# JoshFCooper415/differential_transformer_replication

Measured on AMD Instinct MI355X. Metric: diff-attn fwd+bwd TFLOP/s (% MFMA peak); train tokens/sec at 1/2/4/8 GPUs, higher is better.
Workload: dtype bf16; 1 GPU; cfg2: fused N=2 diff-attention core fwd+bwd (BASELINE configs[1]); batch_per_gpu=8, global_batch=8, heads=16, head_size=64, dv=128, seq_len=4096, n_terms=2, causal=True, parallelism=batch-sharded replicas x1 (no data-path collective)

## Files before the change

### differential_transformer_replication_amd/csrc/attn_kernels.h

```cpp
#pragma once
#include "dta_common.h"
#include "dta_internal.h"
#include "layout_checks.h"

#include <type_traits>
#include <utility>

#ifndef DTA_STAMPS
#define DTA_STAMPS 0
#endif

namespace dta {

template <int NSEG_ = 8>
struct Stamps {
  static constexpr int NSEG = NSEG_;
  unsigned t = 0, s[NSEG] = {};
  __device__ __forceinline__ static unsigned now() {
    unsigned long long v;
    __builtin_amdgcn_sched_barrier(0);
    asm volatile("s_memtime %0\n\ts_waitcnt lgkmcnt(0)" : "=s"(v) : : "memory");
    __builtin_amdgcn_sched_barrier(0);
    return (unsigned)v;
  }
  __device__ __forceinline__ void start() { if constexpr (DTA_STAMPS) t = now(); }
  template <int J>
  __device__ __forceinline__ void lap() {
    if constexpr (DTA_STAMPS) {
      const unsigned n = now();
      s[J] += n - t;
      t = n;
    }
  }
  __device__ __forceinline__ void flush(unsigned long long* out, int wave_id, int lane) {
    if constexpr (DTA_STAMPS) {
      if (out && lane == 0)
#pragma unroll
        for (int j = 0; j < 8; ++j) out[(int64_t)wave_id * 8 + j] = j < NSEG ? s[j] : 0;
    }
  }
};

constexpr int img_cols(int c) {
  int p = 1;
  while (p < c) p <<= 1;
  return p;
}

template <int ROWB>
__device__ __forceinline__ int swz(int r) {
  if constexpr (ROWB >= 256) return ((r & 3) << 2) | ((r >> 2) & 3);
  else if constexpr (ROWB == 128) return (((r >> 1) & 1) << 2) | ((r >> 2) & 3);
  else if constexpr (ROWB == 64) return (r >> 2) & 3;
  else return (r >> 3) & 1;
}

template <class E, int COLS>
struct Img {
  static constexpr int ES = (int)sizeof(E);
  static constexpr int ROWB = COLS * ES;
  static constexpr int CPR = ROWB / 16;
  static_assert(ROWB >= 32 && (ROWB & (ROWB - 1)) == 0, "image rows must be a power of two >= 32 B");
  __device__ static int off(int r, int col) {
    const int byte = col * ES;
    return (r * ROWB + ((((byte >> 4) ^ swz<ROWB>(r)) << 4) | (byte & 15))) / ES;
  }
  using O = Ops<E>;
  using frag = typename O::frag;
  __device__ static frag row(const E* img, int r, int s, int h) {
    if constexpr (ES == 2) return *reinterpret_cast<const frag*>(img + off(r, s * 16 + h * 8));
    else return img[off(r, 2 * s + h)];
  }
  template <class V4>
  __device__ static V4 tr4(const E* img, int r0, int cbase, int lane) {
    const int i = lane & 15;
    const E* p = img + off(r0 + (i >> 2), cbase + ((lane >> 4) & 1) * 16 + (i & 3) * 4);
    s16x4 v = __builtin_amdgcn_ds_read_tr16_b64_v4i16((lds_s16x4*)(p));
    return __builtin_bit_cast(V4, v);
  }
  __device__ static frag tr_perm(const E* img, int rbase, int s, int h, int cbase, int lane) {
    if constexpr (ES == 2) {
      typedef E v4 __attribute__((ext_vector_type(4)));
      v4 lo = tr4<v4>(img, rbase + 16 * s + 4 * h, cbase, lane);
      v4 hi = tr4<v4>(img, rbase + 16 * s + 8 + 4 * h, cbase, lane);
      return __builtin_shufflevector(lo, hi, 0, 1, 2, 3, 4, 5, 6, 7);
    } else {
      return img[off(rbase + (s & 3) + 8 * (s >> 2) + 4 * h, cbase + (lane & 31))];
    }
  }
};

__device__ __forceinline__ void rope_inv4(const float* rope, int64_t row, int hs, int e, float& a0, float& a1,
                                          float& a2, float& a3) {
  const f32x4 t = *reinterpret_cast<const f32x4*>(rope + (row * (hs >> 1) + (e >> 1)) * 2);
  const float b0 = fmaf(a0, t[0], a1 * t[1]), b1 = fmaf(a1, t[0], -a0 * t[1]);
  const float b2 = fmaf(a2, t[2], a3 * t[3]), b3 = fmaf(a3, t[2], -a2 * t[3]);
  a0 = b0; a1 = b1; a2 = b2; a3 = b3;
}

__device__ __forceinline__ uint32_t fmix32(uint32_t x) {
  x ^= x >> 16; x *= 0x85ebca6bu; x ^= x >> 13; x *= 0xc2b2ae35u; x ^= x >> 16;
  return x;
}
__device__ __forceinline__ uint32_t drop_key(uint32_t seed_lo, uint32_t seed_hi, int b, int h, int i, int H, int N) {
  return fmix32(seed_lo ^ fmix32((uint32_t)((b * H + h) * N + i) + seed_hi));
}
__device__ __forceinline__ float drop_mul(uint32_t key, int q, int k, uint32_t thr, float scale) {
  const uint32_t x = fmix32((key + (uint32_t)q * 0x9e3779b1u) ^ ((uint32_t)k * 0x7feb352du));
  return x >= thr ? scale : 0.f;
}

template <class F, int... I>
__device__ __forceinline__ void sfor_impl(F&& f, std::integer_sequence<int, I...>) {
  (f(std::integral_constant<int, I>{}), ...);
}
template <int N, class F>
__device__ __forceinline__ void sfor(F&& f) { sfor_impl(f, std::make_integer_sequence<int, N>{}); }

__device__ __forceinline__ unsigned lds_addr(const void* p) {
  return (unsigned)(uintptr_t)(const __attribute__((address_space(3))) char*)(p);
}

template <int ROWB>
__device__ __forceinline__ int tr_lane(int lane) {
  const int h = (lane >> 5) & 1, i = lane & 15, q = i >> 2;
  const int y = ((lane >> 4) & 1) * 2 + ((i & 3) >> 1);
  int L = (4 * h + q) * ROWB + 16 * (y ^ h) + 8 * (i & 1);
  if constexpr (ROWB >= 256) L += 64 * q;
  else if constexpr (ROWB == 128) L += 64 * (q >> 1);
  return L;
}
template <int ROWB>
__device__ __forceinline__ int row_lane(int lane) {
  const int c = lane & 31, h = (lane >> 5) & 1;
  return c * ROWB + 16 * (h ^ swz<ROWB>(c));
}

typedef long long lds64;
template <int ROWB, int RB, int OFF = 0>
__device__ __forceinline__ void tr_issue(lds64 (&r)[4], unsigned a0, unsigned a1) {
  static_assert(OFF + ROWB * (RB + 24) < 65536, "DS immediate offset");
  asm volatile(
      "ds_read_b64_tr_b16 %0, %4 offset:%6\n\t"
      "ds_read_b64_tr_b16 %1, %5 offset:%7\n\t"
      "ds_read_b64_tr_b16 %2, %4 offset:%8\n\t"
      "ds_read_b64_tr_b16 %3, %5 offset:%9"
      : "=&v"(r[0]), "=&v"(r[1]), "=&v"(r[2]), "=&v"(r[3])
      : "v"(a0), "v"(a1), "i"(OFF + ROWB * RB), "i"(OFF + ROWB * (RB + 8)), "i"(OFF + ROWB * (RB + 16)),
        "i"(OFF + ROWB * (RB + 24)));
}
__device__ __forceinline__ const __attribute__((address_space(3))) char* lds_ptr(unsigned a) {
  return reinterpret_cast<const __attribute__((address_space(3))) char*>((size_t)a);
}
template <class T>
__device__ __forceinline__ T lds_at(unsigned a, int off) {
  return *reinterpret_cast<const __attribute__((address_space(3))) T*>(lds_ptr(a) + off);
}
template <int M>
__device__ __forceinline__ void lgkm_pin(lds64 (&r)[M][4]) {
  asm volatile("s_waitcnt lgkmcnt(0)" ::: "memory");
#pragma unroll
  for (int m = 0; m < M; ++m)
#pragma unroll
    for (int j = 0; j < 4; ++j) asm volatile("" : "+v"(r[m][j]));
}
typedef int i32x4 __attribute__((ext_vector_type(4)));
template <int OFF>
__device__ __forceinline__ void ds128(i32x4& r, unsigned a) {
  static_assert(OFF >= 0 && OFF < 65536, "DS immediate offset");
  asm volatile("ds_read_b128 %0, %1 offset:%2" : "=v"(r) : "v"(a), "i"(OFF));
}
template <int N>
__device__ __forceinline__ void lgkm_wait() {
  asm volatile("s_waitcnt lgkmcnt(%0)" ::"i"(N) : "memory");
}

#ifndef DTA_FWD_PIPE
#define DTA_FWD_PIPE 3
#endif
#ifndef DTA_DQ_PIPE
#define DTA_DQ_PIPE 3
#endif
static_assert(DTA_FWD_PIPE >= 1 && DTA_FWD_PIPE <= 15, "DTA_FWD_PIPE: 1 .. 15 reads ahead");
static_assert(DTA_DQ_PIPE >= 1 && DTA_DQ_PIPE <= 15, "DTA_DQ_PIPE: 1 .. 15 reads ahead");

template <class E, int NSQ, int NKB, int QL, int D, int KOFF, int QOFF, int KROWB>
__device__ __forceinline__ void s_chain_pipe(f32x16 (&sa)[NKB], unsigned bK, unsigned bQ,
                                             const typename Ops<E>::frag* qreg) {
  using frag = typename Ops<E>::frag;
  constexpr int PER = NKB + QL, NR = NSQ * PER;
  constexpr bool KBIG = KOFF + NKB * 32 * KROWB >= 65536, QBIG = QOFF + 1024 >= 65536;
  bK += KBIG ? KOFF : 0;
  bQ += QBIG ? QOFF : 0;
  i32x4 kr[D + 1], qv[QL ? NSQ : 1];
  auto issue = [&](auto J) {
    constexpr int j = decltype(J)::value, st = j / PER, w = j % PER;
    if constexpr (QL && w == 0) ds128<(QBIG ? 0 : QOFF)>(qv[QL ? st : 0], bQ ^ (32 * st));
    else ds128<(KBIG ? 0 : KOFF) + (w - QL) * 32 * KROWB>(kr[(st * NKB + w - QL) % (D + 1)], bK ^ (32 * st));
  };
  sfor<(D < NR ? D : NR)>([&](auto J) { issue(J); });
  sfor<NSQ * NKB>([&](auto C) {
    constexpr int c = decltype(C)::value, st = c / NKB, kb = c % NKB;
    constexpr int j = st * PER + QL + kb;
    constexpr int from = c == 0 ? D : ((c - 1) / NKB) * PER + QL + (c - 1) % NKB + D + 1;
    sfor<NR>([&](auto J2) {
      constexpr int j2 = decltype(J2)::value;
      if constexpr (j2 >= from && j2 <= j + D) issue(std::integral_constant<int, j2>{});
    });
    constexpr int issued = (j + D + 1 < NR ? j + D + 1 : NR);
    lgkm_wait<issued - 1 - j>();
    asm volatile("" : "+v"(kr[c % (D + 1)]));
    frag qb;
    if constexpr (QL) {
      asm volatile("" : "+v"(qv[QL ? st : 0]));
      qb = __builtin_bit_cast(frag, qv[QL ? st : 0]);
    } else {
      qb = qreg[st];
    }
    sa[kb] = Ops<E>::mma(__builtin_bit_cast(frag, kr[c % (D + 1)]), qb, sa[kb]);
  });
}

template <int CNT, int M>
__device__ __forceinline__ void lgkm_pin_n(lds64 (&r)[M][4]) {
  asm volatile("s_waitcnt lgkmcnt(%0)" ::"i"(CNT) : "memory");
#pragma unroll
  for (int m = 0; m < M; ++m)
#pragma unroll
    for (int j = 0; j < 4; ++j) asm volatile("" : "+v"(r[m][j]));
}

template <int ROWB, int RB, int OFF = 0>
__device__ __forceinline__ void tr_load(lds64 (&r)[4], unsigned a0, unsigned a1) {
  typedef short v4s __attribute__((ext_vector_type(4)));
  auto rd = [](unsigned a) {
    return __builtin_bit_cast(lds64, __builtin_amdgcn_ds_read_tr16_b64_v4i16(
        reinterpret_cast<__attribute__((address_space(3))) v4s*>((size_t)a)));
  };
  r[0] = rd(a0 + OFF + ROWB * RB);
  r[1] = rd(a1 + OFF + ROWB * (RB + 8));
  r[2] = rd(a0 + OFF + ROWB * (RB + 16));
  r[3] = rd(a1 + OFF + ROWB * (RB + 24));
}

template <class E>
__device__ __forceinline__ typename Ops<E>::frag tr_frag(const lds64 (&r)[4], int s) {
  typedef short v4s __attribute__((ext_vector_type(4)));
  const v4s lo = __builtin_bit_cast(v4s, r[2 * s]), hi = __builtin_bit_cast(v4s, r[2 * s + 1]);
  return __builtin_bit_cast(typename Ops<E>::frag, __builtin_shufflevector(lo, hi, 0, 1, 2, 3, 4, 5, 6, 7));
}

template <class E, int COLS, int ROWS, int VALID, int NTHR>
__device__ __forceinline__ void stage(E* img, const E* g, int64_t rs, int row0, int rowmax, int tid) {
  using I = Img<E, COLS>;
  constexpr int BYTES = ROWS * I::ROWB;
  if constexpr (VALID == COLS && BYTES % 1024 == 0) {
    constexpr int NI = BYTES / 1024;
    const int wave = tid >> 6, lane = tid & 63;
#pragma unroll
    for (int j0 = 0; j0 < NI; j0 += NTHR / 64) {
      const int j = j0 + wave;
      if (NI % (NTHR / 64) == 0 || j < NI) {
        const int pb = j * 1024 + lane * 16;
        const int r = pb / I::ROWB;
        const int c = ((pb % I::ROWB) >> 4) ^ swz<I::ROWB>(r);
        const int row = min(row0 + r, rowmax);
        const char* src = reinterpret_cast<const char*>(g + (int64_t)row * rs) + c * 16;
        __builtin_amdgcn_global_load_lds(src, (__attribute__((address_space(3))) void*)(reinterpret_cast<char*>(img) + j * 1024),
                                         16, 0, 0);
      }
    }
  } else {
    constexpr int CH = ROWS * I::CPR;
    for (int c = tid; c < CH; c += NTHR) {
      const int r = c / I::CPR, ch = c % I::CPR;
      const int row = row0 + r;
      const bool ok = row <= rowmax && ch * 16 < VALID * I::ES;
      s16x8 v = ok ? *reinterpret_cast<const s16x8*>(reinterpret_cast<const char*>(g + (int64_t)row * rs) + ch * 16)
                   : s16x8{};
      *reinterpret_cast<s16x8*>(reinterpret_cast<char*>(img) + r * I::ROWB + ((ch ^ swz<I::ROWB>(r)) << 4)) = v;
    }
  }
}

template <class E>
__device__ __forceinline__ void rope_frag(typename Ops<E>::frag& f, const float* fr, int t, int col, int HS, int hf) {
  if constexpr (sizeof(E) == 2) {
    const float* q = fr + ((int64_t)t * (HS / 2) + col / 2) * 2;
    const f32x4 a = *reinterpret_cast<const f32x4*>(q), b = *reinterpret_cast<const f32x4*>(q + 4);
    const float cs[4] = {a[0], a[2], b[0], b[2]}, sn[4] = {a[1], a[3], b[1], b[3]};
#pragma unroll
    for (int j = 0; j < 4; ++j) {
      const float x = (float)f[2 * j], y = (float)f[2 * j + 1];
      f[2 * j] = (E)(x * cs[j] - y * sn[j]);
      f[2 * j + 1] = (E)(x * sn[j] + y * cs[j]);
    }
  } else {
    const float* q = fr + ((int64_t)t * (HS / 2) + col / 2) * 2;
    const float c = q[0], sn = q[1];
    const float other = __shfl_xor(f, 32, 64);
    f = hf == 0 ? f * c - other * sn : other * sn + f * c;
  }
}
template <class E, int COLS, int ROWS, int VALID, int NTHR>
__device__ __forceinline__ void rope_lds(E* img, const float* fr, int row0, int T, E* gout, int64_t ors, bool write,
                                         int tid) {
  using I = Img<E, COLS>;
  constexpr int V = 16 / (int)sizeof(E);
  typedef E vec __attribute__((ext_vector_type(V)));
  for (int x = tid; x < ROWS * I::CPR; x += NTHR) {
    const int r = x / I::CPR, ch = x % I::CPR;
    if (ch * V >= VALID) continue;
    const int t = min(row0 + r, T - 1);
    vec* a = reinterpret_cast<vec*>(reinterpret_cast<char*>(img) + r * I::ROWB + ((ch ^ swz<I::ROWB>(r)) << 4));
    vec v = *a;
    const float* q = fr + ((int64_t)t * (VALID / 2) + ch * V / 2) * 2;
#pragma unroll
    for (int j = 0; j < V / 2; ++j) {
      const float c = q[2 * j], sn = q[2 * j + 1];
      const float xx = (float)v[2 * j], yy = (float)v[2 * j + 1];
      v[2 * j] = (E)(xx * c - yy * sn);
      v[2 * j + 1] = (E)(xx * sn + yy * c);
    }
    *a = v;
    if (write && row0 + r < T) *reinterpret_cast<vec*>(gout + (int64_t)(row0 + r) * ors + ch * V) = v;
  }
}

template <class E, int NTHR>
__device__ __forceinline__ void scale_lds(E* a, int n, float s, int tid) {
  constexpr int V = 16 / (int)sizeof(E);
  typedef E vec __attribute__((ext_vector_type(V)));
  for (int e = tid * V; e < n; e += NTHR * V) {
    vec x = *reinterpret_cast<vec*>(a + e);
#pragma unroll
    for (int j = 0; j < V; ++j) x[j] = (E)((float)x[j] * s);
    *reinterpret_cast<vec*>(a + e) = x;
  }
}

template <int N, int NR, int NTHR>
__device__ __forceinline__ void stage_rows(float* dst, const float* src, int64_t bs, int row0, int rowmax, int tid) {
  constexpr int TOT = N * NR;
  constexpr int NI = (TOT + 63) / 64;
  const int wave = tid >> 6, lane = tid & 63;
  for (int j = wave; j < NI; j += NTHR / 64) {
    const int e = j * 64 + lane;
    const int i = min(e / NR, N - 1), r = e % NR;
    const float* s = src + i * bs + min(row0 + r, rowmax);
    __builtin_amdgcn_global_load_lds(s, (__attribute__((address_space(3))) void*)(dst + j * 64), 4, 0, 0);
  }
}

template <int NI, int NW>
__device__ __forceinline__ int pieces(int wave) { return NI / NW + (wave < NI % NW ? 1 : 0); }
template <class E, int COLS, int ROWS, int VALID, int NW>
__device__ __forceinline__ int stage_pieces(int wave) {
  constexpr int BYTES = ROWS * Img<E, COLS>::ROWB;
  if constexpr (VALID == COLS && BYTES % 1024 == 0) return pieces<BYTES / 1024, NW>(wave);
  else return 0;
}
template <int N, int NR, int NW>
__device__ __forceinline__ int rows_pieces(int wave) { return pieces<(N * NR + 63) / 64, NW>(wave); }

__device__ __forceinline__ void wait_vm(int n) {
#define DTA_VM(k) case k: __builtin_amdgcn_s_waitcnt(((k) & 15) | (((k) >> 4) << 14) | (7 << 4) | (15 << 8)); break;
  switch (n) {
    DTA_VM(0) DTA_VM(1) DTA_VM(2) DTA_VM(3) DTA_VM(4) DTA_VM(5) DTA_VM(6) DTA_VM(7) DTA_VM(8) DTA_VM(9)
    DTA_VM(10) DTA_VM(11) DTA_VM(12) DTA_VM(13) DTA_VM(14) DTA_VM(15) DTA_VM(16) DTA_VM(17) DTA_VM(18)
    DTA_VM(19) DTA_VM(20) DTA_VM(21) DTA_VM(22) DTA_VM(23) DTA_VM(24) DTA_VM(25) DTA_VM(26) DTA_VM(27)
    DTA_VM(28) DTA_VM(29) DTA_VM(30) DTA_VM(31)
    default: __builtin_amdgcn_s_waitcnt(0 | (7 << 4) | (15 << 8));
// ... 756 lines not shown
  using QI = Img<E, QP>;
  using KI = Img<E, HSP>;
  using VI = Img<E, DVP>;
  constexpr int BN = CF::BN, BM = CF::BM, NTHR = NW * 64;
  constexpr int KS = O::KSTEP;
  constexpr int NSQ = HS / KS, NSV = DV / KS;
  constexpr int NKB = BN / 32, SPB = 32 / KS, NHB = (HS + 31) / 32;

  extern __shared__ __attribute__((aligned(16))) char smem[];
  E* Qs = reinterpret_cast<E*>(smem);
  constexpr int NS = CF::NS;
  E* Kb = Qs + CF::nQ;
  E* Vb = Kb + NS * CF::nK;

  const int wave = __builtin_amdgcn_readfirstlane(threadIdx.x >> 6);
  int tid = threadIdx.x, lane = tid & 63;
  int hf = lane >> 5, c32 = lane & 31;
  int bx, by, bz, lin;
  lpt_order(bx, by, bz, lin);
  const int qt = gridDim.x - 1 - bx;
  const int hh = by, b = bz;
  const int T = p.T;
  const int q0 = qt * BM, qw0 = q0 + wave * 32;
  int qrow = qw0 + c32;
  const bool rowok = qrow < T;

  const E* gq = reinterpret_cast<const E*>(p.q.p) + b * p.q.sb + hh * p.q.sh;
  const E* gk = reinterpret_cast<const E*>(p.k.p) + b * p.k.sb + hh * p.k.sh;
  const E* gv = reinterpret_cast<const E*>(p.v.p) + b * p.v.sb + hh * p.v.sh;
  const E* gdo = reinterpret_cast<const E*>(p.dout.p) + b * p.dout.sb + hh * p.dout.sh;
  const int64_t gob = b * p.obr.sb + hh * p.obr.sh;

  const int kend = min(T, q0 + BM);
  const int ntiles = (kend + BN - 1) / BN;
  using KR = KvRing<E, HS, N, DV, BN, NW>;
  static_assert(!SRD || (HSP == KR::HSP && DVP == KR::DVP), "descriptor staging fills the kernel's images");
  constexpr bool PRE = SRD && !DROP;
  uint32_t doff[PRE ? KR::MYP : 1];
  if constexpr (PRE) KR::offsets(p.k.st, p.k.si, p.v.st, wave, lane, doff);
  auto stage_kv = [&](int kt, int buf) {
    const int k0 = kt * BN;
    if constexpr (PRE) {
      KR::issue_pre(gk, p.k.st, gv, p.v.st, k0, T, Kb + buf * CF::nK, Vb + buf * CF::nV, wave, doff);
    } else if constexpr (SRD) {
      KR::issue(gk, p.k.st, p.k.si, gv, p.v.st, k0, T, Kb + buf * CF::nK, Vb + buf * CF::nV, wave, lane);
    } else {
#pragma unroll
      for (int i = 0; i < N; ++i)
        stage<E, HSP, BN, HS, NTHR>(Kb + (buf * N + i) * BN * HSP, gk + i * p.k.si, p.k.st, k0, T - 1, tid);
      stage<E, DVP, BN, DV, NTHR>(Vb + buf * CF::nV, gv, p.v.st, k0, T - 1, tid);
    }
  };

  constexpr bool SEED = std::is_same<E, __bf16>::value && !DROP && SRD && !(HS >= 128 && N >= 3);
  constexpr bool SPILLS = sizeof(E) == 2 && (DROP || (HS >= 128 && N >= 3) || (HS >= 192 && N >= 2));
  frag qf[NQR > 0 ? NQR : 1][NQR > 0 ? NSQ : 1], df[NSV];
  float coef[N], lse[N], del[N];
  float dhead = 0.f;
  const int64_t rs = (((int64_t)0 * p.B + b) * p.H + hh) * T + qrow;
  const int64_t bstride = (int64_t)p.B * p.H * T;
#pragma unroll
  for (int s = 0; s < NSV; ++s)
    df[s] = rowok ? O::load_global(gdo + (int64_t)qrow * p.dout.st + s * KS + hf * O::KH) : O::zero();
#pragma unroll
  for (int i = 0; i < N; ++i) {
    coef[i] = p.coef[hh * p.cst + i];
    if (i < NQR) {
#pragma unroll
      for (int s = 0; s < NSQ; ++s)
        qf[i < NQR ? i : 0][s] = rowok ? O::load_global(gq + (int64_t)qrow * p.q.st + i * p.q.si + s * KS + hf * O::KH)
                                       : O::zero();
      if constexpr (SEED) {
#pragma unroll
        for (int s = 0; s < NSQ; ++s)
#pragma unroll
          for (int j = 0; j < 8; ++j) qf[i < NQR ? i : 0][s][j] = (E)((float)qf[i < NQR ? i : 0][s][j] * p.sl2);
      }
    }
    lse[i] = rowok ? p.lse[rs + i * bstride] : 0.f;
    if (p.lsec && rowok && hf == 0) p.lsec[rs + i * bstride] = lse[i] + __builtin_log2f(fabsf(coef[i]));
    float d = 0.f;
    if (rowok) {
#pragma unroll
      for (int s = 0; s < NSV; ++s) {
        const int64_t o = gob + (int64_t)qrow * p.obr.st + i * p.obr.si + s * KS + hf * O::KH;
        if constexpr (sizeof(E) == 2) {
          float ov[8];
          load_ob8(p.obr.p, o, p.ob16, ov);
#pragma unroll
          for (int j = 0; j < 8; ++j) d = fmaf((float)df[s][j], ov[j], d);
        } else {
          d = fmaf(df[s], reinterpret_cast<const float*>(p.obr.p)[o], d);
        }
      }
    }
    d = wave_sum_halves(d);
    del[i] = d;
    const bool kstart = i == 0 || ((p.kstarts >> i) & 1);
    if (kstart) dhead = d;
    if (rowok && hf == 0) p.delta[rs + i * bstride] = DROP ? d : (kstart ? -d : dhead - d);
    float w = (rowok && hf == 0) ? d : 0.f;
#pragma unroll
    for (int o = 32; o > 0; o >>= 1) w += __shfl_xor(w, o, 64);
    if (p.dcoef_part) {
      if (lane == 0 && qw0 < T) p.dcoef_part[(((int64_t)hh * p.cst + i) * p.B + b) * ((T + 31) / 32) + qw0 / 32] = w;
    } else if (lane == 0 && qw0 < T) {
      atomicAdd(p.dcoef + hh * p.cst + i, w);
    }
  }

  if constexpr (!QREG) {
#pragma unroll
    for (int i = NQR; i < N; ++i)
      stage<E, QP, BM, HS, NTHR>(Qs + (i - NQR) * BM * QP, gq + i * p.q.si, p.q.st, q0, T - 1, tid);
  }
  const int tile_pieces = SRD ? KR::pieces(wave)
                              : N * stage_pieces<E, HSP, BN, HS, NW>(wave) + stage_pieces<E, DVP, BN, DV, NW>(wave);
  for (int j = 0; j < NS - 1; ++j)
    if (j < ntiles) stage_kv(j, j);
  wait_vm(tile_pieces * max(0, min(NS - 1, ntiles) - 1));
  lds_barrier();
  frag f_one = O::zero(), f_lse[SEED ? N : 1], f_dp = O::zero();
  float ddel[N];
  if constexpr (SEED) {
    if constexpr (!QREG && N > NQR) {
      scale_lds<E, NTHR>(Qs, CF::nQ, p.sl2, tid);
      lds_barrier();
    }
    if (hf == 0) { f_one[0] = (E)1.f; f_one[1] = (E)1.f; }
#pragma unroll
    for (int i = 0; i < N; ++i) {
      f_lse[i] = seed_frag<E>(lse[i], hf);
      ddel[i] = del[0] - del[i];
    }
    f_dp = seed_frag<E>(-del[0], hf);
  }

  f32x16 dq[N][NHB];
#pragma unroll
  for (int i = 0; i < N; ++i)
#pragma unroll
    for (int d = 0; d < NHB; ++d) dq[i][d] = f32x16{};
  const bool wave_live = qw0 < T;

  int LrV = 0, LrK = 0, LrQ = 0, LtK = 0;
  constexpr int XMAX = 32 * ((NSV > NSQ ? NSV : NSQ) - 1) + 64 * (NHB - 1) + 32;
  constexpr int XM = XMAX < 256 ? 256 : (XMAX < 512 ? 512 : 1024);
  constexpr bool XA = !DROP && SRD && sizeof(E) == 2 && (CF::nQ * (int)sizeof(E)) % XM == 0 &&
                      (CF::nK * (int)sizeof(E)) % XM == 0 && (CF::nV * (int)sizeof(E)) % XM == 0;
  if constexpr (sizeof(E) == 2) {
    LrV = row_lane<VI::ROWB>(lane); LrK = row_lane<KI::ROWB>(lane); LrQ = row_lane<QI::ROWB>(lane);
    LtK = tr_lane<KI::ROWB>(lane);
  }
  Stamps<5> st;
  auto step = [&](int kt, auto MASKED) {
    constexpr bool MASK = decltype(MASKED)::value;
    asm volatile("" : "+v"(lane));
    if constexpr (!DROP && sizeof(E) == 2) {
      asm volatile("" : "+v"(LrV), "+v"(LrK), "+v"(LtK));
      if constexpr (QI::ROWB == KI::ROWB) LrQ = LrK;
      else asm volatile("" : "+v"(LrQ));
    } else if constexpr (sizeof(E) == 2) {
      LrV = row_lane<VI::ROWB>(lane); LrK = row_lane<KI::ROWB>(lane); LrQ = row_lane<QI::ROWB>(lane);
      LtK = tr_lane<KI::ROWB>(lane);
    }
    tid = (wave << 6) + lane; hf = lane >> 5; c32 = lane & 31;
    qrow = qw0 + c32;
    const int buf = kt % NS;
    if (kt + NS - 1 < ntiles) stage_kv(kt + NS - 1, (kt + NS - 1) % NS);
    st.lap<0>();
    const int k0 = kt * BN;
    if (wave_live && k0 <= qw0 + 31) {
      const E* Kc = Kb + buf * CF::nK;
      const E* Vc = Vb + buf * CF::nV;
      unsigned bV = 0, bK = 0, tK = 0;
      if constexpr (XA) {
        bV = LrV + lds_addr(Vc); bK = LrK + lds_addr(Kc); tK = LtK + lds_addr(Kc);
      }
      {
        f32x16 dp[NKB];
        if constexpr (sizeof(E) == 2) {
          const int Lv = LrV;
          const char* vbase = reinterpret_cast<const char*>(Vc);
#pragma unroll
          for (int kb = 0; kb < NKB; ++kb) dp[kb] = SEED ? O::mma(f_one, f_dp, f32x16{}) : f32x16{};
          if constexpr (XA && !SPILLS) {
            constexpr int NIT = NSV * NKB, D = DTA_DQ_PIPE;
            i32x4 vb[D + 1];
            auto issue = [&](auto J) {
              constexpr int j = decltype(J)::value;
              ds128<(j % NKB) * 32 * VI::ROWB>(vb[j % (D + 1)], bV ^ (32 * (j / NKB)));
            };
            sfor<(D < NIT ? D : NIT)>([&](auto J) { issue(J); });
            sfor<NIT>([&](auto J) {
              constexpr int j = decltype(J)::value;
              if constexpr (j + D < NIT) issue(std::integral_constant<int, j + D>{});
              lgkm_wait<(j + D < NIT ? D : NIT - 1 - j)>();
              asm volatile("" : "+v"(vb[j % (D + 1)]));
              dp[j % NKB] = O::mma(__builtin_bit_cast(frag, vb[j % (D + 1)]), df[j / NKB], dp[j % NKB]);
            });
          } else
#pragma unroll
          for (int s = 0; s < NSV; ++s) {
            const int o = Lv ^ (32 * s);
#pragma unroll
            for (int kb = 0; kb < NKB; ++kb) {
              if constexpr (XA) dp[kb] = O::mma(lds_at<frag>(bV ^ (32 * s), kb * 32 * VI::ROWB), df[s], dp[kb]);
              else dp[kb] = O::mma(*reinterpret_cast<const frag*>(vbase + kb * 32 * VI::ROWB + o), df[s], dp[kb]);
            }
          }

        } else {
#pragma unroll
          for (int kb = 0; kb < NKB; ++kb) {
            dp[kb] = f32x16{};
#pragma unroll
            for (int s = 0; s < NSV; ++s) dp[kb] = O::mma(VI::row(Vc, kb * 32 + c32, s, hf), df[s], dp[kb]);
          }
        }
        st.lap<1>();
        sfor<N>([&](auto I_) {
          constexpr int i = decltype(I_)::value;
          const E* Ki = Kc + i * BN * HSP;
          f32x16 sa[NKB];
          if constexpr (XA && !SPILLS) {
            constexpr int QL = i >= NQR ? 1 : 0;
            constexpr int KOFF = i * BN * HSP * (int)sizeof(E), QOFF = (i >= NQR ? i - NQR : 0) * BM * QP * (int)sizeof(E);
#pragma unroll
            for (int kb = 0; kb < NKB; ++kb) sa[kb] = SEED ? O::mma(f_one, f_lse[SEED ? i : 0], f32x16{}) : f32x16{};
            s_chain_pipe<E, NSQ, NKB, QL, DTA_DQ_PIPE, KOFF, QOFF, KI::ROWB>(
                sa, bK, lds_addr(Qs) + wave * 32 * QI::ROWB + LrQ, qf[i < NQR ? i : 0]);
          } else if constexpr (sizeof(E) == 2) {
            const int Lr = LrK;
            const char* kbase = reinterpret_cast<const char*>(Ki);
            const char* qbase = reinterpret_cast<const char*>(Qs + (i >= NQR ? i - NQR : 0) * BM * QP) +
                                wave * 32 * QI::ROWB;
            const int Lq = LrQ;
#pragma unroll
            for (int kb = 0; kb < NKB; ++kb) sa[kb] = SEED ? O::mma(f_one, f_lse[SEED ? i : 0], f32x16{}) : f32x16{};
#pragma unroll
            for (int s = 0; s < NSQ; ++s) {
              frag qb;
              if (i < NQR) qb = qf[i < NQR ? i : 0][s];
              else qb = *reinterpret_cast<const frag*>(qbase + (Lq ^ (32 * s)));
#pragma unroll
              for (int kb = 0; kb < NKB; ++kb) {
                if constexpr (XA)
                  sa[kb] = O::mma(lds_at<frag>(bK ^ (32 * s), (i * BN * HSP) * (int)sizeof(E) + kb * 32 * KI::ROWB), qb,
                                  sa[kb]);
                else
                  sa[kb] = O::mma(*reinterpret_cast<const frag*>(kbase + kb * 32 * KI::ROWB + (Lr ^ (32 * s))), qb, sa[kb]);
              }
            }
          } else {
#pragma unroll
            for (int kb = 0; kb < NKB; ++kb) {
              sa[kb] = f32x16{};
#pragma unroll
              for (int s = 0; s < NSQ; ++s) {
                frag qb;
                if (i < NQR) qb = qf[i < NQR ? i : 0][s];
                else qb = QI::row(Qs + (i >= NQR ? i - NQR : 0) * BM * QP, wave * 32 + c32, s, hf);
                sa[kb] = O::mma(KI::row(Ki, kb * 32 + c32, s, hf), qb, sa[kb]);
              }
            }
          }
          const float li = lse[i], ci = coef[i], cdi = coef[i] * del[i];
          const int lim = min(qrow, T - 1) - k0 - 4 * hf;
          if constexpr (SEED) {
            const float dd = ddel[i];
#pragma unroll
            for (int kb = 0; kb < NKB; ++kb)
#pragma unroll
              for (int r0 = 0; r0 < 16; r0 += DTA_DQ_EXPG) {
                float pr[DTA_DQ_EXPG];
#pragma unroll
                for (int u = 0; u < DTA_DQ_EXPG; ++u) {
                  const int r = r0 + u;
                  float arg = sa[kb][r];
                  if constexpr (MASK) arg = (kb * 32 + (r & 3) + 8 * (r >> 2) > lim) ? -INFINITY : arg;
                  pr[u] = exp2_fast(arg);
                }
#pragma unroll
                for (int u = 0; u < DTA_DQ_EXPG; ++u) {
                  const int r = r0 + u;
                  sa[kb][r] = i == 0 ? pr[u] * dp[kb][r] : pr[u] * (dp[kb][r] + dd);
                }
              }
          } else {
          uint32_t dkey = 0;
          if constexpr (DROP) dkey = drop_key(p.drop_seed_lo, p.drop_seed_hi, b, hh, p.br0 + i, p.H, p.cst);
#pragma unroll
          for (int kb = 0; kb < NKB; ++kb)
#pragma unroll
            for (int r = 0; r < 16; ++r) {
              float arg = fmaf(sa[kb][r], p.sl2, li);
              if constexpr (MASK) arg = (kb * 32 + (r & 3) + 8 * (r >> 2) > lim) ? -INFINITY : arg;
              float cm = ci;
              if constexpr (DROP)
                cm *= drop_mul(dkey, qrow, k0 + kb * 32 + (r & 3) + 8 * (r >> 2) + 4 * hf, p.drop_thr, p.drop_scale);
              sa[kb][r] = exp2_fast(arg) * fmaf(cm, dp[kb][r], -cdi);
            }
          }
          if constexpr (sizeof(E) == 2) {
            const unsigned kbse = lds_addr(Ki);
            const int Lk = LtK;
            sfor<NHB>([&](auto D) {
              constexpr int d = decltype(D)::value;
              lds64 r[NKB][4];
              const unsigned a0 = XA ? (tK ^ (64 * d)) + (unsigned)(i * BN * HSP * (int)sizeof(E)) : kbse + (Lk ^ (64 * d));
              const unsigned a1 = XA ? (tK ^ (64 * d + 32)) + (unsigned)(i * BN * HSP * (int)sizeof(E))
                                     : kbse + (Lk ^ (64 * d + 32));
              if constexpr (SPILLS) {
                sfor<NKB>([&](auto KB) { tr_load<KI::ROWB, 32 * decltype(KB)::value>(r[decltype(KB)::value], a0, a1); });
              } else {
                sfor<NKB>([&](auto KB) { tr_issue<KI::ROWB, 32 * decltype(KB)::value>(r[decltype(KB)::value], a0, a1); });
                lgkm_pin<NKB>(r);
              }
#pragma unroll
              for (int kb = 0; kb < NKB; ++kb) {
                dq[i][d] = O::mma(tr_frag<E>(r[kb], 0), O::template pack<0>(sa[kb]), dq[i][d]);
                dq[i][d] = O::mma(tr_frag<E>(r[kb], 1), O::template pack<1>(sa[kb]), dq[i][d]);
              }
            });
          } else {
#pragma unroll
            for (int d = 0; d < NHB; ++d)
#pragma unroll
              for (int kb = 0; kb < NKB; ++kb)
#pragma unroll
                for (int s = 0; s < SPB; ++s)
                  dq[i][d] = O::mma(KI::tr_perm(Ki, kb * 32, s, hf, d * 32, lane), sa[kb][s], dq[i][d]);
          }
        });
      }
    }
    st.lap<2>();
    wait_vm(tile_pieces * max(0, min(NS - 2, ntiles - 2 - kt)));
    st.lap<3>();
    lds_barrier();
    st.lap<4>();
  };
  st.start();
  const int nfull = min(ntiles, min((q0 + 1) / BN, T / BN));
  for (int kt = 0; kt < nfull; ++kt) step(kt, std::false_type{});
  for (int kt = nfull; kt < ntiles; ++kt) step(kt, std::true_type{});
  st.flush(p.stamps, lin * NW + wave, lane);

  if (qw0 >= T) return;
  constexpr bool BNC = sizeof(E) == 2 && NHB % 2 == 0 && CF::bytes >= NW * 8192;
  if constexpr (BNC) {
    if (OUTF32 || t5_aligned16(p.dq, sizeof(E))) {
      float* reg = reinterpret_cast<float*>(smem) + wave * 2048;
      const int nrows = min(32, T - qw0);
      const int rrow = min(qrow, T - 1);
#pragma unroll
      for (int i = 0; i < N; ++i) {
        const float sc = SEED ? p.scale * coef[i] : p.scale;
        auto val = [&](int d, int g) {
          float a0 = dq[i][d][4 * g] * sc, a1 = dq[i][d][4 * g + 1] * sc;
          float a2 = dq[i][d][4 * g + 2] * sc, a3 = dq[i][d][4 * g + 3] * sc;
          if (p.rope) rope_inv4(p.rope, rrow, HS, d * 32 + 8 * g + 4 * hf, a0, a1, a2, a3);
          return f32x4{a0, a1, a2, a3};
        };
        if constexpr (OUTF32)
          bounce_store<float, NHB>(reg, lane, val, p.dq32 + ((((int64_t)b * T + qw0) * p.H + hh) * p.cst + i) * HS,
                                   (int64_t)p.H * p.cst * HS, nrows);
        else
          bounce_store<E, NHB>(reg, lane, val, reinterpret_cast<E*>(p.dq.p) + b * p.dq.sb + (int64_t)qw0 * p.dq.st +
                                                   hh * p.dq.sh + i * p.dq.si, p.dq.st, nrows);
      }
      return;
    }
  }
  if (!rowok) return;
#pragma unroll
  for (int i = 0; i < N; ++i)
#pragma unroll
    for (int d = 0; d < NHB; ++d)
#pragma unroll
      for (int g = 0; g < 4; ++g) {
        const int e = d * 32 + 8 * g + 4 * hf;
        if (e >= HS) continue;
        const float sc = SEED ? p.scale * coef[i] : p.scale;
        float a0 = dq[i][d][4 * g] * sc, a1 = dq[i][d][4 * g + 1] * sc;
        float a2 = dq[i][d][4 * g + 2] * sc, a3 = dq[i][d][4 * g + 3] * sc;
        if (p.rope) rope_inv4(p.rope, qrow, HS, e, a0, a1, a2, a3);
        if constexpr (OUTF32) {
          store4<float>(p.dq32 + ((((int64_t)b * T + qrow) * p.H + hh) * p.cst + i) * HS + e, a0, a1, a2, a3);
        } else {
          E* gdq = reinterpret_cast<E*>(p.dq.p) + b * p.dq.sb + (int64_t)qrow * p.dq.st + hh * p.dq.sh + i * p.dq.si;
          store4<E>(gdq + e, a0, a1, a2, a3);
        }
      }
}

template <class E, int HS, int N, int DV, int NW, bool DELTA, int BQ_ = 32, bool ROWS = true>
struct TileRing {
  static constexpr int ES = (int)sizeof(E), BQ = BQ_;
  static constexpr int NP = (N * BQ + 63) / 64 * 64;
  static constexpr int HSP = img_cols(HS), DVP = img_cols(DV);
  static constexpr int QB = BQ * HSP * ES, DB = BQ * DVP * ES;
  static constexpr int OFF_D = N * QB, OFF_L = OFF_D + DB, OFF_G = OFF_L + NP * 4;
  static constexpr int SB = ROWS ? OFF_G + NP * 4 : OFF_L;
  static constexpr int PQ = N * QB / 1024, PD = DB / 1024, PL = NP / 64;
  static constexpr int NPC = PQ + PD + (ROWS ? (DELTA ? 2 : 1) * PL : 0);
  static constexpr int MYP = (NPC + NW - 1) / NW;
  static constexpr bool ok = ES == 2 && HS >= 32 && QB % 1024 == 0 && DB % 1024 == 0;

  __device__ static int pieces(int wave) { return NPC / NW + (wave < NPC % NW ? 1 : 0); }

  __device__ static uint32_t offq(const BwdParams& p, int j, int lane) {
    using QI = Img<E, HSP>;
    const int i = j / (QB / 1024), pb = (j % (QB / 1024)) * 1024 + lane * 16;
    const int r = pb / QI::ROWB;
    int c = ((pb % QI::ROWB) >> 4) ^ swz<QI::ROWB>(r);
    if constexpr (HSP != HS) c = c * 16 < HS * ES ? c : 0;
    return (uint32_t)(r * (uint32_t)(p.q.st * ES) + (uint32_t)(i * p.q.si * ES) + c * 16);
  }
  __device__ static uint32_t offd(const BwdParams& p, int j, int lane) {
    using DI = Img<E, DVP>;
    const int pb = (j - PQ) * 1024 + lane * 16;
    const int r = pb / DI::ROWB;
    int c = ((pb % DI::ROWB) >> 4) ^ swz<DI::ROWB>(r);
    if constexpr (DVP != DV) c = c * 16 < DV * ES ? c : 0;
    return (uint32_t)(r * (uint32_t)(p.dout.st * ES) + c * 16);
  }
  __device__ static uint32_t offr(int j, int lane, int64_t bstride) {
    const int e = ((j - PQ - PD) % PL) * 64 + lane;
    const int i = min(e / BQ, N - 1), r = e % BQ;
    return (uint32_t)((i * (uint32_t)bstride + r) * 4);
  }
  __device__ static void offsets(const BwdParams& p, int64_t bstride, int wave, int lane, uint32_t (&off)[MYP]) {
    sfor<MYP>([&](auto U) {
      constexpr int u = decltype(U)::value;
      const int j = u * NW + wave;
      if constexpr ((u + 1) * NW <= PQ) off[u] = offq(p, j, lane);
      else if constexpr (u * NW >= PQ && (u + 1) * NW <= PQ + PD) off[u] = offd(p, j, lane);
      else off[u] = j < PQ ? offq(p, j, lane) : (j < PQ + PD ? offd(p, j, lane) : (j < NPC ? offr(j, lane, bstride) : 0u));
    });
  }
  __device__ static void issue_pre(const BwdParams& p, const E* gq, const E* gdo, const float* lse, const float* delta,
                                   int64_t bstride, int q0, int T, char* st0, int wave, const uint32_t (&off)[MYP]) {
    const int rows = T - q0;
    const E* bq = gq + (int64_t)q0 * p.q.st;
    const E* bd = gdo + (int64_t)q0 * p.dout.st;
    const uint32_t nq = (uint32_t)rows * (uint32_t)(p.q.st * ES), nd = (uint32_t)rows * (uint32_t)(p.dout.st * ES);
    const uint32_t nl = (uint32_t)(((N - 1) * bstride + rows) * 4);
    sfor<MYP>([&](auto U) {
      constexpr int u = decltype(U)::value;
      const int j = u * NW + wave;
      if constexpr ((u + 1) * NW <= PQ) {
        buf_lds16(bq, nq, st0 + j * 1024, off[u]);
      } else if constexpr (u * NW >= PQ && (u + 1) * NW <= PQ + PD) {
        buf_lds16(bd, nd, st0 + OFF_D + (j - PQ) * 1024, off[u]);
      } else {
        if (j < PQ) buf_lds16(bq, nq, st0 + j * 1024, off[u]);
        else if (j < PQ + PD) buf_lds16(bd, nd, st0 + OFF_D + (j - PQ) * 1024, off[u]);
        else if (j < PQ + PD + PL) buf_lds4(lse + q0, nl, st0 + OFF_L + (j - PQ - PD) * 256, off[u]);
        else if (j < NPC) buf_lds4(delta + q0, nl, st0 + OFF_G + (j - PQ - PD - PL) * 256, off[u]);
      }
    });
  }
};

inline bool ring_layout_ok(const BwdParams& p, int es) {
  return dma_rows_ok(p.T, p.q.st, p.q.si, p.N, p.HS, es) && dma_rows_ok(p.T, p.dout.st, 0, 1, p.DV, es) &&
         dma_rowvecs_ok(p.N, p.B, p.H, p.T);
}


template <class E, int HS, int N, int DV, int NW, bool PR = false, bool GRX = false>
struct DkdvCfg {
  static constexpr int LIMB = PR ? 80 * 1024 : 160 * 1024;
  static constexpr int BK = NW * 32;
  static constexpr int HSP = img_cols(HS < 32 ? 32 : HS), KP = img_cols(HS), DVP = img_cols(DV);
  static constexpr int BQ = 32;
  static constexpr int NP = (N * BQ + 63) / 64 * 64;
  static constexpr int nQ = N * BQ * HSP;
  static constexpr int nD = BQ * DVP;
  static constexpr int nK = N * BK * KP;
  static constexpr int RB = 2 * NP * 4;
  static constexpr bool GR = GRX;
  static constexpr int NS = ring_stages_lim(nK * (int)sizeof(E), (nQ + nD) * (int)sizeof(E) + (GR ? 0 : RB), LIMB);
  static constexpr int bytes = (nK + NS * nQ + NS * nD) * (int)sizeof(E) + (GR ? 0 : NS * RB);
};

template <int HS, int N, int DV>
struct DkdvSplit {
  static constexpr int HSB = (HS < 32 ? 32 : HS + 31) / 32 * 32;
  static constexpr bool fused = (N * HSB / 2 + DV / 2) <= 160;
};

template <class E, int HS, int N, int DV, bool NP = false>
// ... 692 lines not shown
```

Measured before the change: 579.0 TFLOP/s.

## Interleave dS exp/scale work with S and dQ MFMA chains in backward dQ kernel

Adds a kb-major ordering mode to the S-chain pipeline with a callback hook, so the exp/scale (dS) computation for each key block runs between MFMAs instead of as a separate phase. The dQ accumulation is rewritten into a double-buffered transposed-load pipeline that also interleaves the next block's dS work between MFMA pairs. The aim is to hide VALU exp work and LDS read latency behind matrix ops in the specialised configuration (NKB=2, 4 waves, head size 64). Timing stamps gain more segments. The cost is more complex scheduling and possible register pressure.

```diff
diff --git a/differential_transformer_replication_amd/csrc/attn_kernels.h b/differential_transformer_replication_amd/csrc/attn_kernels.h
--- a/differential_transformer_replication_amd/csrc/attn_kernels.h
+++ b/differential_transformer_replication_amd/csrc/attn_kernels.h
@@ -15,6 +15,7 @@
 template <int NSEG_ = 8>
 struct Stamps {
   static constexpr int NSEG = NSEG_;
+  static constexpr int SLOTS = NSEG <= 8 ? 8 : 16;
   unsigned t = 0, s[NSEG] = {};
   __device__ __forceinline__ static unsigned now() {
     unsigned long long v;
@@ -36,7 +37,16 @@
     if constexpr (DTA_STAMPS) {
       if (out && lane == 0)
 #pragma unroll
-        for (int j = 0; j < 8; ++j) out[(int64_t)wave_id * 8 + j] = j < NSEG ? s[j] : 0;
+        for (int j = 0; j < SLOTS; ++j) out[(int64_t)wave_id * SLOTS + j] = j < NSEG ? s[j] : 0;
+    }
+  }
+  template <int J>
+  __device__ __forceinline__ void lap_on(float v) {
+    if constexpr (DTA_STAMPS) {
+      __builtin_amdgcn_sched_barrier(0);
+      const int x = __builtin_amdgcn_readfirstlane(__builtin_bit_cast(int, v));
+      asm volatile("" ::"s"(x));
+      lap<J>();
     }
   }
 };
@@ -184,9 +194,13 @@
 static_assert(DTA_FWD_PIPE >= 1 && DTA_FWD_PIPE <= 15, "DTA_FWD_PIPE: 1 .. 15 reads ahead");
 static_assert(DTA_DQ_PIPE >= 1 && DTA_DQ_PIPE <= 15, "DTA_DQ_PIPE: 1 .. 15 reads ahead");
 
-template <class E, int NSQ, int NKB, int QL, int D, int KOFF, int QOFF, int KROWB>
+struct NoMid {
+  template <class KB, class ST>
+  __device__ __forceinline__ void operator()(KB, ST) const {}
+};
+template <class E, int NSQ, int NKB, int QL, int D, int KOFF, int QOFF, int KROWB, bool KBM = false, class F = NoMid>
 __device__ __forceinline__ void s_chain_pipe(f32x16 (&sa)[NKB], unsigned bK, unsigned bQ,
-                                             const typename Ops<E>::frag* qreg) {
+                                             const typename Ops<E>::frag* qreg, F mid = F{}) {
   using frag = typename Ops<E>::frag;
   constexpr int PER = NKB + QL, NR = NSQ * PER;
   constexpr bool KBIG = KOFF + NKB * 32 * KROWB >= 65536, QBIG = QOFF + 1024 >= 65536;
@@ -194,15 +208,22 @@
   bQ += QBIG ? QOFF : 0;
   i32x4 kr[D + 1], qv[QL ? NSQ : 1];
   auto issue = [&](auto J) {
-    constexpr int j = decltype(J)::value, st = j / PER, w = j % PER;
-    if constexpr (QL && w == 0) ds128<(QBIG ? 0 : QOFF)>(qv[QL ? st : 0], bQ ^ (32 * st));
-    else ds128<(KBIG ? 0 : KOFF) + (w - QL) * 32 * KROWB>(kr[(st * NKB + w - QL) % (D + 1)], bK ^ (32 * st));
+    constexpr int j = decltype(J)::value;
+    constexpr bool first = j < NSQ * (1 + QL);
+    constexpr int st = !KBM ? j / PER : (first ? j / (1 + QL) : (j - NSQ * (1 + QL)) % NSQ);
+    constexpr int w = !KBM ? j % PER - QL : (first ? j % (1 + QL) - QL : 1 + (j - NSQ * (1 + QL)) / NSQ);
+    if constexpr (w < 0) ds128<(QBIG ? 0 : QOFF)>(qv[QL ? st : 0], bQ ^ (32 * st));
+    else ds128<(KBIG ? 0 : KOFF) + w * 32 * KROWB>(kr[(KBM ? w * NSQ + st : st * NKB + w) % (D + 1)], bK ^ (32 * st));
+  };
+  auto kread = [](int c) {
+    if constexpr (KBM) return c < NSQ ? c * (1 + QL) + QL : NSQ * QL + c;
+    else return (c / NKB) * PER + QL + c % NKB;
   };
   sfor<(D < NR ? D : NR)>([&](auto J) { issue(J); });
   sfor<NSQ * NKB>([&](auto C) {
-    constexpr int c = decltype(C)::value, st = c / NKB, kb = c % NKB;
-    constexpr int j = st * PER + QL + kb;
-    constexpr int from = c == 0 ? D : ((c - 1) / NKB) * PER + QL + (c - 1) % NKB + D + 1;
+    constexpr int c = decltype(C)::value, st = KBM ? c % NSQ : c / NKB, kb = KBM ? c / NSQ : c % NKB;
+    constexpr int j = kread(c);
+    constexpr int from = c == 0 ? D : kread(c - 1) + D + 1;
     sfor<NR>([&](auto J2) {
       constexpr int j2 = decltype(J2)::value;
       if constexpr (j2 >= from && j2 <= j + D) issue(std::integral_constant<int, j2>{});
@@ -218,6 +239,7 @@
       qb = qreg[st];
     }
     sa[kb] = Ops<E>::mma(__builtin_bit_cast(frag, kr[c % (D + 1)]), qb, sa[kb]);
+    if constexpr (KBM && kb >= 1) mid(std::integral_constant<int, kb>{}, std::integral_constant<int, st>{});
   });
 }
 
@@ -1280,7 +1302,9 @@
     LrV = row_lane<VI::ROWB>(lane); LrK = row_lane<KI::ROWB>(lane); LrQ = row_lane<QI::ROWB>(lane);
     LtK = tr_lane<KI::ROWB>(lane);
   }
-  Stamps<5> st;
+  constexpr bool TRC = XA && !SPILLS && sizeof(E) == 2 && NKB == 2 && NW == 4 && QRH == 1 && HS == 64;
+  constexpr bool KBM = TRC && SEED;
+  Stamps<9> st;
   auto step = [&](int kt, auto MASKED) {
     constexpr bool MASK = decltype(MASKED)::value;
     asm volatile("" : "+v"(lane));
@@ -1351,13 +1375,42 @@
           constexpr int i = decltype(I_)::value;
           const E* Ki = Kc + i * BN * HSP;
           f32x16 sa[NKB];
+          const float li = lse[i], ci = coef[i], cdi = coef[i] * del[i];
+          const int lim = min(qrow, T - 1) - k0 - 4 * hf;
+          auto ds_group = [&](int kb, int r0) {
+            const float dd = ddel[i];
+            float pr[DTA_DQ_EXPG];
+#pragma unroll
+            for (int u = 0; u < DTA_DQ_EXPG; ++u) {
+              const int r = r0 + u;
+              float arg = sa[kb][r];
+              if constexpr (MASK) arg = (kb * 32 + (r & 3) + 8 * (r >> 2) > lim) ? -INFINITY : arg;
+              pr[u] = exp2_fast(arg);
+            }
+#pragma unroll
+            for (int u = 0; u < DTA_DQ_EXPG; ++u) {
+              const int r = r0 + u;
+              sa[kb][r] = i == 0 ? pr[u] * dp[kb][r] : pr[u] * (dp[kb][r] + dd);
+            }
+          };
+          auto ds_slot = [&](int kb, int m, int M) {
+            constexpr int NG = 16 / DTA_DQ_EXPG;
+#pragma unroll
+            for (int g = m * NG / M; g < (m + 1) * NG / M; ++g) ds_group(kb, g * DTA_DQ_EXPG);
+          };
           if constexpr (XA && !SPILLS) {
             constexpr int QL = i >= NQR ? 1 : 0;
             constexpr int KOFF = i * BN * HSP * (int)sizeof(E), QOFF = (i >= NQR ? i - NQR : 0) * BM * QP * (int)sizeof(E);
 #pragma unroll
             for (int kb = 0; kb < NKB; ++kb) sa[kb] = SEED ? O::mma(f_one, f_lse[SEED ? i : 0], f32x16{}) : f32x16{};
-            s_chain_pipe<E, NSQ, NKB, QL, DTA_DQ_PIPE, KOFF, QOFF, KI::ROWB>(
-                sa, bK, lds_addr(Qs) + wave * 32 * QI::ROWB + LrQ, qf[i < NQR ? i : 0]);
+            if constexpr (KBM) {
+              s_chain_pipe<E, NSQ, NKB, QL, DTA_DQ_PIPE, KOFF, QOFF, KI::ROWB, true>(
+                  sa, bK, lds_addr(Qs) + wave * 32 * QI::ROWB + LrQ, qf[i < NQR ? i : 0],
+                  [&](auto KB, auto ST) { ds_slot(decltype(KB)::value - 1, decltype(ST)::value, NSQ); });
+            } else {
+              s_chain_pipe<E, NSQ, NKB, QL, DTA_DQ_PIPE, KOFF, QOFF, KI::ROWB>(
+                  sa, bK, lds_addr(Qs) + wave * 32 * QI::ROWB + LrQ, qf[i < NQR ? i : 0]);
+            }
           } else if constexpr (sizeof(E) == 2) {
             const int Lr = LrK;
             const char* kbase = reinterpret_cast<const char*>(Ki);
@@ -1393,28 +1446,14 @@
               }
             }
           }
-          const float li = lse[i], ci = coef[i], cdi = coef[i] * del[i];
-          const int lim = min(qrow, T - 1) - k0 - 4 * hf;
-          if constexpr (SEED) {
-            const float dd = ddel[i];
+          st.template lap<2>();
+          st.template lap_on<3>(sa[NKB - 1][15]);
+          if constexpr (KBM) {
+          } else if constexpr (SEED) {
 #pragma unroll
             for (int kb = 0; kb < NKB; ++kb)
 #pragma unroll
-              for (int r0 = 0; r0 < 16; r0 += DTA_DQ_EXPG) {
-                float pr[DTA_DQ_EXPG];
-#pragma unroll
-                for (int u = 0; u < DTA_DQ_EXPG; ++u) {
-                  const int r = r0 + u;
-                  float arg = sa[kb][r];
-                  if constexpr (MASK) arg = (kb * 32 + (r & 3) + 8 * (r >> 2) > lim) ? -INFINITY : arg;
-                  pr[u] = exp2_fast(arg);
-                }
-#pragma unroll
-                for (int u = 0; u < DTA_DQ_EXPG; ++u) {
-                  const int r = r0 + u;
-                  sa[kb][r] = i == 0 ? pr[u] * dp[kb][r] : pr[u] * (dp[kb][r] + dd);
-                }
-              }
+              for (int r0 = 0; r0 < 16; r0 += DTA_DQ_EXPG) ds_group(kb, r0);
           } else {
           uint32_t dkey = 0;
           if constexpr (DROP) dkey = drop_key(p.drop_seed_lo, p.drop_seed_hi, b, hh, p.br0 + i, p.H, p.cst);
@@ -1430,7 +1469,34 @@
               sa[kb][r] = exp2_fast(arg) * fmaf(cm, dp[kb][r], -cdi);
             }
           }
-          if constexpr (sizeof(E) == 2) {
+          st.template lap<4>();
+          if constexpr (TRC) {
+            constexpr int G = NHB * NKB;
+            constexpr unsigned ioff = (unsigned)(i * BN * HSP * (int)sizeof(E));
+            lds64 r[2][1][4];
+            frag pk[NKB][2];
+            auto issue = [&](auto G_) {
+              constexpr int g = decltype(G_)::value, kb = KBM ? g / NHB : g % NKB, d = KBM ? g % NHB : g / NKB;
+              tr_issue<KI::ROWB, 32 * kb>(r[g & 1][0], (tK ^ (64 * d)) + ioff, (tK ^ (64 * d + 32)) + ioff);
+            };
+            issue(std::integral_constant<int, 0>{});
+            if constexpr (G > 1) issue(std::integral_constant<int, 1>{});
+            sfor<G>([&](auto G_) {
+              constexpr int g = decltype(G_)::value, kb = KBM ? g / NHB : g % NKB, d = KBM ? g % NHB : g / NKB;
+              if constexpr (d == 0) {
+                pk[kb][0] = O::template pack<0>(sa[kb]);
+                pk[kb][1] = O::template pack<1>(sa[kb]);
+              }
+              lgkm_pin_n<4 * ((g + 2 < G ? g + 2 : G) - 1 - g), 1>(r[g & 1]);
+              st.template lap<5>();
+              dq[i][d] = O::mma(tr_frag<E>(r[g & 1][0], 0), pk[kb][0], dq[i][d]);
+              if constexpr (KBM && kb + 1 < NKB) ds_slot(kb + 1, 2 * d, 2 * NHB);
+              dq[i][d] = O::mma(tr_frag<E>(r[g & 1][0], 1), pk[kb][1], dq[i][d]);
+              if constexpr (KBM && kb + 1 < NKB) ds_slot(kb + 1, 2 * d + 1, 2 * NHB);
+              st.template lap<6>();
+              if constexpr (g + 2 < G) issue(std::integral_constant<int, g + 2>{});
+            });
+          } else if constexpr (sizeof(E) == 2) {
             const unsigned kbse = lds_addr(Ki);
             const int Lk = LtK;
             sfor<NHB>([&](auto D) {
@@ -1445,11 +1511,13 @@
                 sfor<NKB>([&](auto KB) { tr_issue<KI::ROWB, 32 * decltype(KB)::value>(r[decltype(KB)::value], a0, a1); });
                 lgkm_pin<NKB>(r);
               }
+              st.template lap<5>();
 #pragma unroll
               for (int kb = 0; kb < NKB; ++kb) {
                 dq[i][d] = O::mma(tr_frag<E>(r[kb], 0), O::template pack<0>(sa[kb]), dq[i][d]);
                 dq[i][d] = O::mma(tr_frag<E>(r[kb], 1), O::template pack<1>(sa[kb]), dq[i][d]);
               }
+              st.template lap<6>();
             });
           } else {
 #pragma unroll
@@ -1463,11 +1531,11 @@
         });
       }
     }
-    st.lap<2>();
+    st.lap<6>();
     wait_vm(tile_pieces * max(0, min(NS - 2, ntiles - 2 - kt)));
-    st.lap<3>();
+    st.lap<7>();
     lds_barrier();
-    st.lap<4>();
+    st.lap<8>();
   };
   st.start();
   const int nfull = min(ntiles, min((q0 + 1) / BN, T / BN));
```

Result: no change. 582.7 TFLOP/s (median of 6 runs) (+0.6%).
